# IC3Net/IC3Net

Hardware: AMD Instinct MI355X
Metric: env-steps/sec (agents x envs x steps), rollout hot path (higher is better)
Workload: dtype f32

## Files before the change

### ic3net_amd/csrc/bptt_kernels.hip

```cpp
#include <hip/hip_runtime.h>

#include <algorithm>
#include <vector>

#include "enc_bwd.hpp"
#include "ic3_common.hpp"
#include "ps_common.hpp"

extern "C" int ic3_lstm_gates_backward_given(const float* gates, float* xh, int ldx, const float* h_prev, const void* lstm_wp3_bwd,
                                             const float* c_prev, const float* dh, const float* dc, float* dgates, float* dc_prev,
                                             float* dbias_partials, int accumulate, float* dxh, const float* row_live,
                                             const float* row_keep, const float* dhead, const float* w_heads, int OT, int R, int H,
                                             ic3_stream stream);

namespace ic3 {

typedef float bp_f32x2 __attribute__((ext_vector_type(2)));
typedef float bp_f32x4 __attribute__((ext_vector_type(4)));
typedef float bp_f32x16 __attribute__((ext_vector_type(16)));

__device__ __forceinline__ __amdgpu_buffer_rsrc_t bp_rsrc(const void* base, long long bytes)
{
    const uint32_t n = bytes <= 0 ? 0u : (bytes > 0xffffffffll ? 0xffffffffu : (uint32_t)bytes);
    return __builtin_amdgcn_make_buffer_rsrc(const_cast<void*>(base), 0, n, 0x00020000);
// ... 493 lines not shown
        IC3_HIP(hipGetLastError());
        const int n3 = 2 * H * 4 * H;
        hipLaunchKernelGGL(wgrad_reduce_kernel, dim3((n3 + 255) / 256), dim3(256), 0, s, scratch, ks, n3, dW, accumulate);
        IC3_HIP(hipGetLastError());
        return ks;
    }
    const size_t lds = (size_t)2 * 16 * (2 * H + 128) * sizeof(float);
    if (H == 128) {
        IC3_HIP(ensure_dynamic_lds(reinterpret_cast<const void*>(lstm_wgrad_kernel<128>), lds));
        hipLaunchKernelGGL((lstm_wgrad_kernel<128>), dim3(ks, 4), dim3(256), lds, s, a);
    } else {
        IC3_HIP(ensure_dynamic_lds(reinterpret_cast<const void*>(lstm_wgrad_kernel<64>), lds));
        hipLaunchKernelGGL((lstm_wgrad_kernel<64>), dim3(ks, 2), dim3(256), lds, s, a);
    }
    IC3_HIP(hipGetLastError());
    const int n = 2 * H * 4 * H;
    hipLaunchKernelGGL(wgrad_reduce_kernel, dim3((n + 255) / 256), dim3(256), 0, s, scratch, ks, n, dW, accumulate);
    IC3_HIP(hipGetLastError());
    return ks;
}

extern "C" int ic3_bptt_backward_supported(const ic3_env* env, int H)
{
    using namespace ic3;
    if (!env || (H != 64 && H != 128 && H != 256) || env->dims.N > 64) return 0;
    EncBwdPlan pl;
    if (env->kind == IC3_ENV_PP) {
        const ic3_pp_cfg& c = env->pp;
        const int W = 2 * c.vision + 1;
        pl = enc_bwd_plan(c.E, env->dims.N, c.N + c.nprey, H, c.dim * c.dim, 2 * W * W);
    } else {
        const ic3_tj_cfg& c = env->tj;
        const int WW = env->dims.window * env->dims.window, hdr = c.vocab_type ? 4 : 2;
        pl = enc_bwd_plan(c.E, c.N, c.N, H, env->dims.grid_h * env->dims.grid_w, hdr + WW);
    }
    return pl.csplit ? 1 : 0;
}

namespace ic3 {
struct BpttSide {
    hipStream_t stream = nullptr;
    hipEvent_t fork = nullptr, join = nullptr;
};
static BpttSide* bptt_side()
{
    static BpttSide side[64];
    int dev = 0;
    if (hipGetDevice(&dev) != hipSuccess || dev < 0 || dev >= 64) return nullptr;
    BpttSide& sd = side[dev];
    if (!sd.stream) {
        if (hipStreamCreateWithFlags(&sd.stream, hipStreamNonBlocking) != hipSuccess) return nullptr;
        if (hipEventCreateWithFlags(&sd.fork, hipEventDisableTiming) != hipSuccess ||
            hipEventCreateWithFlags(&sd.join, hipEventDisableTiming) != hipSuccess)
            return nullptr;
    }
    return &sd;
}
}

extern "C" int ic3_bptt_first_chain_envs(int E, int N)
{
    if (E < 128 || N <= 0) return E;
    return (E / 2) & ~63;
}

extern "C" int ic3_bptt_backward(ic3_env* env, const ic3_bptt* b, ic3_stream stream)
{
    using namespace ic3;
    if (!env || !b) return fail(-22, "ic3_bptt_backward: null argument");
    if (b->struct_size != sizeof(ic3_bptt))
        return fail(-22, "ic3_bptt_backward: ic3_bptt has " + std::to_string(b->struct_size) + " bytes, this library's has " +
                             std::to_string(sizeof(ic3_bptt)) + " (header / library version mismatch)");
    const int T = b->T, E = b->E, N = b->N, H = b->H;
    if (T <= 0 || E <= 0 || N <= 0 || E != env->dims.E || N != env->dims.N)
        return fail(-22, "ic3_bptt_backward: T, E, N must be positive and E, N the handle's");
    if (!ic3_bptt_backward_supported(env, H)) return fail(-38, "ic3_bptt_backward: hid_size 64 / 128 / 256, <= 64 agents, a grid whose encoder backward runs in its partial-sums form");
    if (b->OT < 1 || b->OT > 16) return fail(-22, "ic3_bptt_backward: 1 <= OT <= 16");
    if (!b->gates || !b->hs || !b->cs || !b->dhead || !b->snaps || !b->lstm_wp3_bwd || !b->w_heads || !b->dh || !b->dc || !b->dxh ||
        !b->dbias_partials || !b->enc_work)
        return fail(-22, "ic3_bptt_backward: null argument");
    if (!b->comm_zero && (!b->c_weight || !b->dcw_partials)) return fail(-22, "ic3_bptt_backward: C.weight and its partials");
    if (b->dxh_step && (b->dxh_step < (long long)E * N * 2 * H || ic3_env_encode_backward_window_work(env, H) <= 0))
        return fail(-22, "ic3_bptt_backward: dxh_step >= E * N * 2 * hid_size, on a configuration with ic3_env_encode_backward_window");
    const long long R = (long long)E * N;
    hipStream_t s = (hipStream_t)stream;
    const int E1 = (b->two_chains && b->dxh_step) ? ic3_bptt_first_chain_envs(E, N) : E;
    const int nch = E1 < E ? 2 : 1;
    BpttSide* side = nch == 2 ? bptt_side() : nullptr;
    if (nch == 2 && !side) return fail(-12, "ic3_bptt_backward: no second stream");
    if (nch == 2) {
        IC3_HIP(hipEventRecord(side->fork, s));
        IC3_HIP(hipStreamWaitEvent(side->stream, side->fork, 0));
    }
    int enc_first = b->enc_first;
    for (int t = T - 1; t >= 0; --t) {
        for (int ch = 0; ch < nch; ++ch) {
            const int e0 = ch ? E1 : 0, Ec = ch ? E - E1 : E1;
            const size_t r0 = (size_t)e0 * N, Rc = (size_t)Ec * N;
            hipStream_t sc = ch ? side->stream : s;
            ic3_stream scv = (ic3_stream)sc;
            float* dh = b->dh + r0 * H;
            float* dc = b->dc + r0 * H;
            const bool detached = b->detach_gap > 0 && (t + 1) % b->detach_gap == 0;
            float* g = b->gates + ((size_t)t * R + r0) * 4 * H;
            float* dxh = b->dxh + (size_t)t * (size_t)b->dxh_step + r0 * 2 * H;
            if (b->gate_events && ch == 0) IC3_HIP(hipEventRecord((hipEvent_t)b->gate_events[2 * t], sc));
            int rc = ic3_lstm_gates_backward_given(g, nullptr, 0, nullptr, b->lstm_wp3_bwd, b->cs + ((size_t)t * R + r0) * H,
                                                   detached ? nullptr : dh, detached ? nullptr : dc, g,
                                                   dc, b->dbias_partials + (r0 / 64) * 4 * H, 1, dxh,
                                                   b->row_live ? b->row_live + (size_t)t * R + r0 : nullptr,
                                                   b->row_keep ? b->row_keep + (size_t)t * R + r0 : nullptr,
                                                   b->dhead + ((size_t)t * R + r0) * b->OT, b->w_heads, b->OT, (int)Rc, H, scv);
            if (rc < 0) return rc;
            if (b->gate_events && ch == 0) IC3_HIP(hipEventRecord((hipEvent_t)b->gate_events[2 * t + 1], sc));
            const float* out_scale = (b->row_keep && t > 0) ? b->row_keep + (size_t)(t - 1) * R + r0 : nullptr;
            float* dcw = b->dcw_partials;
            if (dcw && ch) dcw += (size_t)ic3_comm_backward_partials(E1, N) * H * H;
            rc = ic3_comm_backward(dxh, 2 * H, b->hs + ((size_t)t * R + r0) * H, (b->alive && b->alive[t]) ? b->alive[t] + r0 : nullptr,
                                   (b->gate && b->gate[t]) ? b->gate[t] + r0 : nullptr, b->c_weight, out_scale, dh, dcw, 1, Ec, N, H,
                                   b->mode_avg, b->comm_zero, scv);
            if (rc < 0) return rc;
        }
        if (b->dxh_step) continue;
        int rc = ic3_env_encode_backward_accumulate(env, b->snaps + (size_t)t * b->snap_words, b->dxh, 2 * H, H, b->enc_work,
                                                    enc_first, stream);
        if (rc < 0) return rc;
        enc_first = 0;
    }
    if (nch == 2) {
        IC3_HIP(hipEventRecord(side->join, side->stream));
        IC3_HIP(hipStreamWaitEvent(s, side->join, 0));
    }
    if (b->dxh_step)
        return ic3_env_encode_backward_window(env, b->snaps, b->snap_words, T, b->dxh, 2 * H, b->dxh_step, H, b->enc_work, enc_first,
                                              stream);
    return 0;
}

namespace ic3 {

struct RnnBwdArgs {
    const float* dh_in;
    const float* h;
    const float* dhead;
    const float* w_heads;
    const float* a2;
    const float* out_scale;
    float* dz;
    float* dh_out;
    float* db_part;
    int R, OT, tiles, accumulate;
};

template <int H>
__global__ __launch_bounds__(4 * H, (H <= 64) ? 2 : 1) void rnn_tanh_bwd_kernel(const RnnBwdArgs a)
{
    constexpr int NT = 4 * H, H4 = H / 4, LDA = H + 4, LDA4 = LDA / 4, CB = H / 32, RPP = NT / H4, PER = 64 / RPP;
    static_assert(RPP * PER == 64 && NT / 64 == 2 * CB, "tile split");
    IC3_DYNAMIC_LDS(float, smem);
    const bp_f32x4* const Bf4 = reinterpret_cast<const bp_f32x4*>(smem);
    float* const Dz = smem + H * H;
    bp_f32x4* const Dz4 = reinterpret_cast<bp_f32x4*>(Dz);
    float* const Wh = Dz + 64 * LDA;
    const bp_f32x4* const Wh4 = reinterpret_cast<const bp_f32x4*>(Wh);
    float* const Sd = Wh + 16 * H;
    const int tid = threadIdx.x, lane = tid & 63, w = tid >> 6, li = lane & 31, lh = lane >> 5;
    const int cb = w % CB, rb = w / CB;
    const int c4 = tid % H4, rg = tid / H4;
    const int OT = a.OT;
    for (int i = tid; i < H * H; i += NT) {
        const int k = i / H, col = i - k * H;
        smem[(((k >> 3) * 2 + ((k >> 2) & 1)) * H + col) * 4 + (k & 3)] = a.a2[i];
    }
    for (int i = tid; i < OT * H; i += NT) Wh[i] = a.w_heads[i];
    bp_f32x4 bsum = { 0.f, 0.f, 0.f, 0.f };
    __syncthreads();
    for (int tile = blockIdx.x; tile < a.tiles; tile += gridDim.x) {
        const long long r0 = (long long)tile * 64;
        const int rows = (a.R - r0) < 64 ? (int)(a.R - r0) : 64;
        const __amdgpu_buffer_rsrc_t rdi = bp_rsrc(a.dh_in ? a.dh_in + r0 * H : a.h, a.dh_in ? (long long)rows * H * 4 : 0);
        const __amdgpu_buffer_rsrc_t rh = bp_rsrc(a.h + r0 * H, (long long)rows * H * 4);
        const __amdgpu_buffer_rsrc_t rd = bp_rsrc(a.dhead + r0 * OT, (long long)rows * OT * 4);
        const __amdgpu_buffer_rsrc_t rz = bp_rsrc(a.dz + r0 * H, (long long)rows * H * 4);
        bp_f32x4 dv[PER], hv[PER];
#pragma unroll
        for (int i = 0; i < PER; ++i) {
            const int off = ((rg + RPP * i) * H + 4 * c4) * 4;
            dv[i] = bp_load4(rdi, off);
            hv[i] = bp_load4(rh, off);
        }
        for (int i = tid; i < 64 * OT; i += NT) Sd[i] = bp_load1(rd, i * 4);
        __syncthreads();
#pragma unroll
        for (int i = 0; i < PER; ++i) {
            const int row = rg + RPP * i;
            bp_f32x4 v = dv[i];
            for (int o = 0; o < OT; ++o) v += Sd[row * OT + o] * Wh4[o * H4 + c4];
            const bp_f32x4 z = v * (1.0f - hv[i] * hv[i]);
            bsum += z;
            Dz4[row * LDA4 + c4] = z;
            __builtin_amdgcn_raw_buffer_store_b128(__builtin_bit_cast(ps_u32x4, z), rz, (row * H + 4 * c4) * 4, 0, 0);
        }
        __syncthreads();
        bp_f32x16 acc;
#pragma unroll
        for (int i = 0; i < 16; ++i) acc[i] = 0.0f;
#pragma unroll 4
        for (int kb = 0; kb < H / 8; ++kb) {
            const bp_f32x4 a4 = Dz4[(32 * rb + li) * LDA4 + 2 * kb + lh];
// ... 246 lines not shown
```

### ic3net_amd/csrc/gates_bwd.hip

```cpp
#include <hip/hip_runtime.h>

#include "ic3_common.hpp"

namespace ic3 {

typedef float gb_f32x4 __attribute__((ext_vector_type(4)));
typedef float gb_f32x16 __attribute__((ext_vector_type(16)));
typedef unsigned int gb_u32x4 __attribute__((ext_vector_type(4)));

struct GatesBwdArgs {
    float* xh;
    const float* h_prev;
    const float* wq;
    const void* wq3;
    const float* bias;
    const float* c_prev;
    const float* dh;
    const float* dc;
    float* dgates;
    float* dc_prev;
    float* dbias;
    int ldx, R, accumulate;
    const void* wb3;
    float* dxh;
    const float* gates;
    const float* row_live;
    const float* row_keep;
    const float* dhead;
    const float* w_heads;
    int OT;
};

__device__ __forceinline__ __amdgpu_buffer_rsrc_t gb_rsrc(const void* base, long long bytes)
{
    const uint32_t n = bytes <= 0 ? 0u : (bytes > 0xffffffffll ? 0xffffffffu : (uint32_t)bytes);
    return __builtin_amdgcn_make_buffer_rsrc(const_cast<void*>(base), 0, n, 0x00020000);
}
__device__ __forceinline__ gb_f32x4 gb_load4(__amdgpu_buffer_rsrc_t r, int voff, int soff)
{
    return __builtin_bit_cast(gb_f32x4, __builtin_amdgcn_raw_buffer_load_b128(r, voff, soff, 0));
}
__device__ __forceinline__ float gb_load1(__amdgpu_buffer_rsrc_t r, int voff, int soff)
{
    return __builtin_bit_cast(float, __builtin_amdgcn_raw_buffer_load_b32(r, voff, soff, 0));
}
__device__ __forceinline__ void gb_store1(float v, __amdgpu_buffer_rsrc_t r, int voff, int soff)
{
    __builtin_amdgcn_raw_buffer_store_b32(__builtin_bit_cast(int, v), r, voff, soff, 0);
}

__device__ __forceinline__ void gb_mfma(gb_f32x16& acc, float x, float y)
{
    acc = __builtin_amdgcn_mfma_f32_32x32x2f32(x, y, acc, 0, 0, 0);
}

typedef __bf16 gb_bf16x2 __attribute__((ext_vector_type(2)));
typedef float gb_f32x2 __attribute__((ext_vector_type(2)));
__device__ __forceinline__ void gb_split_pair(gb_f32x2 x, unsigned& p1, unsigned& p2, unsigned& p3)
{
    const gb_bf16x2 h1 = __builtin_convertvector(x, gb_bf16x2);
    const gb_f32x2 r1 = x - __builtin_convertvector(h1, gb_f32x2);
    const gb_bf16x2 h2 = __builtin_convertvector(r1, gb_bf16x2);
    const gb_f32x2 r2 = r1 - __builtin_convertvector(h2, gb_f32x2);
    const gb_bf16x2 h3 = __builtin_convertvector(r2, gb_bf16x2);
    p1 = __builtin_bit_cast(unsigned, h1);
    p2 = __builtin_bit_cast(unsigned, h2);
    p3 = __builtin_bit_cast(unsigned, h3);
}
__device__ __forceinline__ void gb_split_frag(gb_f32x4 x0, gb_f32x4 x1, gb_u32x4 (&out)[3])
{
    unsigned p[3][4];
    gb_split_pair(gb_f32x2{ x0[0], x0[1] }, p[0][0], p[1][0], p[2][0]);
    gb_split_pair(gb_f32x2{ x0[2], x0[3] }, p[0][1], p[1][1], p[2][1]);
    gb_split_pair(gb_f32x2{ x1[0], x1[1] }, p[0][2], p[1][2], p[2][2]);
    gb_split_pair(gb_f32x2{ x1[2], x1[3] }, p[0][3], p[1][3], p[2][3]);
#pragma unroll
    for (int pl = 0; pl < 3; ++pl) out[pl] = gb_u32x4{ p[pl][0], p[pl][1], p[pl][2], p[pl][3] };
}
__device__ __forceinline__ void gb_mfma_bf16(gb_f32x16& acc, gb_u32x4 x, gb_u32x4 y)
{
    typedef __bf16 gb_bf16x8 __attribute__((ext_vector_type(8)));
    acc = __builtin_amdgcn_mfma_f32_32x32x16_bf16(__builtin_bit_cast(gb_bf16x8, x), __builtin_bit_cast(gb_bf16x8, y), acc, 0, 0, 0);
}

template <int H, int SPLIT = 0, int GIVEN = 0>
__global__ __launch_bounds__(2 * H, (H <= 128) ? 2 : 1) void lstm_gates_bwd_kernel(const GatesBwdArgs a)
{
    static_assert(!GIVEN || SPLIT == 1, "recorded gates: the split instantiation (its dx product)");
    constexpr int K = 2 * H, LDA = K + 4, LDA4 = LDA / 4, NT = 2 * H, KB = K / 8, K4 = K / 4, RING = 8;
    static_assert(KB % 2 == 0 && KB >= 4, "K / 8 must be even");
    IC3_DYNAMIC_LDS(float, smem);
    float* const As = smem;
    gb_f32x4* const As4 = reinterpret_cast<gb_f32x4*>(smem);
    float* const slb = As + 64 * LDA;
    float* const sdh = slb + 4 * H;
    const int tid = threadIdx.x, lane = tid & 63, w = tid >> 6, li = lane & 31, lh = lane >> 5;
    const int col = 32 * w + li;
    const long long r0 = (long long)blockIdx.x * 64;
    const int rows = (int)((a.R - r0) < 64 ? (a.R - r0) : 64);

    if constexpr (GIVEN != 0) {
        if (a.dhead) {
            const __amdgpu_buffer_rsrc_t rdd = gb_rsrc(a.dhead + r0 * a.OT, (long long)rows * a.OT * 4);
            for (int idx = tid; idx < 64 * 16; idx += NT) {
                const int row = idx >> 4, o = idx & 15;
                sdh[idx] = o < a.OT ? gb_load1(rdd, (row * a.OT + o) * 4, 0) : 0.0f;
            }
        }
        if (a.xh && a.h_prev) {
            const __amdgpu_buffer_rsrc_t rx = gb_rsrc(a.xh + r0 * a.ldx, ((long long)(rows - 1) * a.ldx + K) * 4);
            const __amdgpu_buffer_rsrc_t rhp = gb_rsrc(a.h_prev + r0 * H, (long long)rows * H * 4);
            constexpr int H4 = H / 4, PERH = 64 * H4 / NT;
#pragma unroll
            for (int i = 0; i < PERH; ++i) {
                const int idx = tid + i * NT, row = idx / H4, c4 = idx - row * H4;
                gb_f32x4 v = gb_load4(rhp, (row * H + 4 * c4) * 4, 0);
                if (a.row_live) v *= (row < rows ? a.row_live[r0 + row] : 0.0f);
                __builtin_amdgcn_raw_buffer_store_b128(__builtin_bit_cast(gb_u32x4, v), rx, (row * a.ldx + H + 4 * c4) * 4, 0, 0);
            }
        }
    } else {
        const __amdgpu_buffer_rsrc_t rx = gb_rsrc(a.xh + r0 * a.ldx, ((long long)(rows - 1) * a.ldx + K) * 4);
        constexpr int PER = 64 * K4 / NT;
        const __amdgpu_buffer_rsrc_t rhp = gb_rsrc(a.h_prev ? a.h_prev + r0 * H : a.xh, a.h_prev ? (long long)rows * H * 4 : 0);
        const bool from_h = a.h_prev != nullptr;
        gb_f32x4 v[PER];
#pragma unroll
        for (int i = 0; i < PER; ++i) {
            const int idx = tid + i * NT, row = idx / K4, c4 = idx - row * K4;
            if (from_h && c4 >= H / 4) {
                v[i] = gb_load4(rhp, (row * H + 4 * c4 - H) * 4, 0);
                __builtin_amdgcn_raw_buffer_store_b128(__builtin_bit_cast(gb_u32x4, v[i]), rx, (row * a.ldx + 4 * c4) * 4, 0, 0);
            } else {
                v[i] = gb_load4(rx, (row * a.ldx + 4 * c4) * 4, 0);
            }
        }
        if (tid < H) reinterpret_cast<gb_f32x4*>(slb)[tid] = reinterpret_cast<const gb_f32x4*>(a.bias)[tid];
#pragma unroll
        for (int i = 0; i < PER; ++i) {
            const int idx = tid + i * NT, row = idx / K4, c4 = idx - row * K4;
            As4[row * LDA4 + c4] = v[i];
        }
    }
    const int voff = (4 * lh * H + col) * 4;
    float cold[2][16];
    const __amdgpu_buffer_rsrc_t rc = gb_rsrc(a.c_prev + r0 * H, (long long)rows * H * 4);
    if constexpr (SPLIT == 0) {
#pragma unroll
        for (int rt = 0; rt < 2; ++rt)
#pragma unroll
            for (int reg = 0; reg < 16; ++reg)
                cold[rt][reg] = gb_load1(rc, voff, (32 * rt + (reg & 3) + 8 * (reg >> 2)) * H * 4);
    }
    gb_f32x16 acc[2][4];
#pragma unroll
    for (int rt = 0; rt < 2; ++rt)
#pragma unroll
        for (int gt = 0; gt < 4; ++gt)
#pragma unroll
            for (int i = 0; i < 16; ++i) acc[rt][gt][i] = 0.0f;
    if constexpr (GIVEN != 0) {
    } else if constexpr (SPLIT != 0) {
        constexpr int KB16 = K / 16, NWv = H / 32;
        const __amdgpu_buffer_rsrc_t rg3 = gb_rsrc(a.wq3, (long long)3 * K * 4 * H * 2);
        const int g3lane = (w * 64 + lane) * 16;
        constexpr int GSTRIDE = NWv * 64 * 16;
        auto wq3 = [&](int pl, int kb, int gt) {
            return __builtin_amdgcn_raw_buffer_load_b128(rg3, g3lane, ((pl * KB16 + kb) * 4 + gt) * GSTRIDE, 0);
        };
        gb_u32x4 bq[3][4];
#pragma unroll
        for (int pl = 0; pl < 3; ++pl)
#pragma unroll
            for (int gt = 0; gt < 4; ++gt) bq[pl][gt] = wq3(pl, 0, gt);
        __syncthreads();
        auto block3 = [&](auto refill_c, int kb) {
            constexpr bool REFILL = decltype(refill_c)::value;
            gb_u32x4 ap[2][3];
            {
                const gb_f32x4* s0 = As4 + li * LDA4 + 4 * kb + 2 * lh;
                const gb_f32x4* s1 = As4 + (32 + li) * LDA4 + 4 * kb + 2 * lh;
                gb_split_frag(s0[0], s0[1], ap[0]);
                gb_split_frag(s1[0], s1[1], ap[1]);
            }
#pragma unroll
            for (int pb = 0; pb < 3; ++pb)
#pragma unroll
                for (int gt = 0; gt < 4; ++gt) {
#pragma unroll
                    for (int pa = 2; pa >= 0; --pa) {
                        gb_mfma_bf16(acc[0][gt], ap[0][pa], bq[pb][gt]);
                        gb_mfma_bf16(acc[1][gt], ap[1][pa], bq[pb][gt]);
                    }
                    if constexpr (REFILL) bq[pb][gt] = wq3(pb, kb + 1, gt);
                    __builtin_amdgcn_sched_barrier(0);
                }
        };
#pragma unroll 1
        for (int kb = 0; kb < KB16 - 1; ++kb) block3(std::true_type{}, kb);
        block3(std::false_type{}, KB16 - 1);
        __builtin_amdgcn_sched_barrier(0);
    } else {
        const __amdgpu_buffer_rsrc_t rgw = gb_rsrc(a.wq, (long long)K * 4 * H * 4);
        const int glane = (4 * lh * H + col) * 16;
        auto wq = [&](int kb, int j) { return gb_load4(rgw, glane, (8 * kb + j) * (H * 16)); };
        gb_f32x4 wk[RING];
    #pragma unroll
        for (int i = 0; i < RING; ++i) wk[i] = wq(i >> 2, i & 3);
        __syncthreads();
        auto block = [&](auto sb_c, auto refill_c, int kb) {
            constexpr int SB = decltype(sb_c)::value;
            constexpr bool REFILL = decltype(refill_c)::value;
            const gb_f32x4 a0 = As4[li * LDA4 + 2 * kb + lh];
            const gb_f32x4 a1 = As4[(32 + li) * LDA4 + 2 * kb + lh];
    #pragma unroll
            for (int j = 0; j < 4; ++j) {
    #pragma unroll
                for (int gt = 0; gt < 4; ++gt) {
                    gb_mfma(acc[0][gt], a0[j], wk[SB + j][gt]);
                    gb_mfma(acc[1][gt], a1[j], wk[SB + j][gt]);
                }
                if constexpr (REFILL) wk[SB + j] = wq(kb + RING / 4, j);
                __builtin_amdgcn_sched_barrier(0);
            }
        };
        constexpr std::integral_constant<int, 0> s0{};
        constexpr std::integral_constant<int, 4> s1{};
    #pragma unroll 1
        for (int kb = 0; kb < KB - 2; kb += 2) {
            block(s0, std::true_type{}, kb);
            block(s1, std::true_type{}, kb + 1);
        }
        block(s0, std::false_type{}, KB - 2);
        block(s1, std::false_type{}, KB - 1);
        __builtin_amdgcn_sched_barrier(0);
    }

    const float bi = GIVEN ? 0.f : slb[col], bf = GIVEN ? 0.f : slb[H + col], bg = GIVEN ? 0.f : slb[2 * H + col], bo = GIVEN ? 0.f : slb[3 * H + col];
    const bool dx = SPLIT != 0 && a.dxh != nullptr;
    float keep_g[2][16], keep_o[2][16];
    const bool heads_in = GIVEN != 0 && a.dhead != nullptr;
    if (dx || heads_in) __syncthreads();
    float wh[16] = {};
    if constexpr (GIVEN != 0) {
        if (heads_in) {
            const __amdgpu_buffer_rsrc_t rwh = gb_rsrc(a.w_heads, (long long)a.OT * H * 4);
#pragma unroll
            for (int o = 0; o < 16; ++o) wh[o] = gb_load1(rwh, (o * H + col) * 4, 0);
        }
    }
    const long long nrec = (long long)rows * H * 4;
    const __amdgpu_buffer_rsrc_t rdh = gb_rsrc(a.dh ? a.dh + r0 * H : a.c_prev, a.dh ? nrec : 0);
    const __amdgpu_buffer_rsrc_t rdc = gb_rsrc(a.dc ? a.dc + r0 * H : a.c_prev, a.dc ? nrec : 0);
    const __amdgpu_buffer_rsrc_t rdp = gb_rsrc(a.dc_prev + r0 * H, nrec);
    const __amdgpu_buffer_rsrc_t rdg = gb_rsrc(a.dgates + r0 * 4 * H, 4 * nrec);
    const int goff = (4 * lh * 4 * H + col) * 4;
    const __amdgpu_buffer_rsrc_t rgin = gb_rsrc(GIVEN ? a.gates + r0 * 4 * H : a.c_prev, GIVEN ? 4 * nrec : 0);
    const bool cuts = GIVEN != 0 && (a.row_live != nullptr || a.row_keep != nullptr);
    const __amdgpu_buffer_rsrc_t rlive = gb_rsrc(a.row_live ? a.row_live + r0 : a.c_prev, a.row_live ? (long long)rows * 4 : 0);
    const __amdgpu_buffer_rsrc_t rkeep = gb_rsrc(a.row_keep ? a.row_keep + r0 : a.c_prev, a.row_keep ? (long long)rows * 4 : 0);
    float si = 0.f, sf = 0.f, sg = 0.f, so = 0.f;
#pragma unroll
    for (int rt = 0; rt < 2; ++rt) {
        float dhv[16], dcv[16], gin[GIVEN ? 4 : 1][16];
#pragma unroll
        for (int reg = 0; reg < 16; ++reg) {
            const int lc = 32 * rt + (reg & 3) + 8 * (reg >> 2);
            dhv[reg] = gb_load1(rdh, voff, lc * H * 4);
            dcv[reg] = gb_load1(rdc, voff, lc * H * 4);
            if constexpr (SPLIT != 0) cold[rt][reg] = gb_load1(rc, voff, lc * H * 4);
            if constexpr (GIVEN != 0) {
#pragma unroll
                for (int k = 0; k < 4; ++k) gin[k][reg] = gb_load1(rgin, goff, lc * 4 * H * 4 + k * H * 4);
            }
        }
#pragma unroll
        for (int reg = 0; reg < 16; ++reg) {
            const int lc = 32 * rt + (reg & 3) + 8 * (reg >> 2);
            float i, f, gt, o;
            if constexpr (GIVEN != 0) {
                i = gin[0][reg], f = gin[1][reg], gt = gin[2][reg], o = gin[3][reg];
                if (heads_in) {
                    const gb_f32x4* dr = reinterpret_cast<const gb_f32x4*>(sdh + (lc + 4 * lh) * 16);
                    float s = dhv[reg];
#pragma unroll
                    for (int q = 0; q < 4; ++q) {
                        if (4 * q >= a.OT) break;
                        const gb_f32x4 dv = dr[q];
                        s = __builtin_fmaf(dv[0], wh[4 * q], s);
                        s = __builtin_fmaf(dv[1], wh[4 * q + 1], s);
                        s = __builtin_fmaf(dv[2], wh[4 * q + 2], s);
                        s = __builtin_fmaf(dv[3], wh[4 * q + 3], s);
                    }
                    dhv[reg] = s;
                }
                if (cuts) {
                    const int lrow = lc + 4 * lh;
                    if (a.row_live) cold[rt][reg] *= gb_load1(rlive, lrow * 4, 0);
                    if (a.row_keep) dcv[reg] *= gb_load1(rkeep, lrow * 4, 0);
                }
            } else {
                i = fast_sigmoid(acc[rt][0][reg] + bi), f = fast_sigmoid(acc[rt][1][reg] + bf);
                gt = fast_tanh(acc[rt][2][reg] + bg), o = fast_sigmoid(acc[rt][3][reg] + bo);
            }
            const float c0 = cold[rt][reg];
            const float tc = fast_tanh(__builtin_fmaf(f, c0, i * gt));
            const float dct = dcv[reg] + dhv[reg] * o * (1.0f - tc * tc);
            const float di = dct * gt * i * (1.0f - i), df = dct * c0 * f * (1.0f - f);
            const float dg = dct * i * (1.0f - gt * gt), dO = dhv[reg] * tc * o * (1.0f - o);
            gb_store1(di, rdg, goff, lc * 4 * H * 4);
            gb_store1(df, rdg, goff, lc * 4 * H * 4 + H * 4);
            gb_store1(dg, rdg, goff, lc * 4 * H * 4 + 2 * H * 4);
            gb_store1(dO, rdg, goff, lc * 4 * H * 4 + 3 * H * 4);
            gb_store1(dct * f, rdp, voff, lc * H * 4);
            if constexpr (SPLIT != 0) {
                if (dx) {
                    const int lr = lc + 4 * lh;
                    As[lr * LDA + col] = di;
                    As[lr * LDA + H + col] = df;
                    keep_g[rt][reg] = dg;
                    keep_o[rt][reg] = dO;
                }
            }
            si += di;
            sf += df;
            sg += dg;
            so += dO;
        }
    }
    if constexpr (SPLIT != 0) {
        if (dx) {
            constexpr int KB16B = 4 * H / 16, NCT = 2 * H / 32, KBH = K / 16;
            const __amdgpu_buffer_rsrc_t rwb = gb_rsrc(a.wb3, (long long)3 * 4 * H * 2 * H * 2);
            const int wu = __builtin_amdgcn_readfirstlane(w);
            auto wb = [&](int pl, int kg, int ct) __attribute__((always_inline)) {
                return __builtin_amdgcn_raw_buffer_load_b128(rwb, lane * 16, ((pl * KB16B + kg) * NCT + 2 * wu + ct) * 1024, 0);
            };
            gb_u32x4 bq2[3][2];
#pragma unroll
            for (int pl = 0; pl < 3; ++pl)
#pragma unroll
                for (int ct = 0; ct < 2; ++ct) bq2[pl][ct] = wb(pl, 0, ct);
#pragma unroll
            for (int rt = 0; rt < 2; ++rt)
#pragma unroll
                for (int ct = 0; ct < 2; ++ct)
#pragma unroll
                    for (int i = 0; i < 16; ++i) acc[rt][ct][i] = 0.0f;
            auto blockdx = [&](int kb, int kg) __attribute__((always_inline)) {
                gb_u32x4 ap[2][3];
                const gb_f32x4* s0 = As4 + li * LDA4 + 4 * kb + 2 * lh;
                const gb_f32x4* s1 = As4 + (32 + li) * LDA4 + 4 * kb + 2 * lh;
                gb_split_frag(s0[0], s0[1], ap[0]);
                gb_split_frag(s1[0], s1[1], ap[1]);
#pragma unroll
                for (int pb = 0; pb < 3; ++pb)
#pragma unroll
                    for (int ct = 0; ct < 2; ++ct) {
#pragma unroll
                        for (int pa = 2; pa >= 0; --pa) {
                            gb_mfma_bf16(acc[0][ct], ap[0][pa], bq2[pb][ct]);
                            gb_mfma_bf16(acc[1][ct], ap[1][pa], bq2[pb][ct]);
                        }
                        if (kg + 1 < KB16B) bq2[pb][ct] = wb(pb, kg + 1, ct);
                        __builtin_amdgcn_sched_barrier(0);
                    }
            };
            __syncthreads();
#pragma unroll 1
            for (int kb = 0; kb < KBH; ++kb) blockdx(kb, kb);
            __syncthreads();
#pragma unroll
            for (int rt = 0; rt < 2; ++rt)
#pragma unroll
                for (int reg = 0; reg < 16; ++reg) {
                    const int lr = 32 * rt + (reg & 3) + 8 * (reg >> 2) + 4 * lh;
                    As[lr * LDA + col] = keep_g[rt][reg];
                    As[lr * LDA + H + col] = keep_o[rt][reg];
                }
            __syncthreads();
#pragma unroll 1
            for (int kb = 0; kb < KBH; ++kb) blockdx(kb, KBH + kb);
            const __amdgpu_buffer_rsrc_t rdx = gb_rsrc(a.dxh + r0 * K, (long long)rows * K * 4);
#pragma unroll
            for (int rt = 0; rt < 2; ++rt)
#pragma unroll
                for (int ct = 0; ct < 2; ++ct)
#pragma unroll
                    for (int reg = 0; reg < 16; ++reg) {
                        const int lr = 32 * rt + (reg & 3) + 8 * (reg >> 2) + 4 * lh;
                        gb_store1(acc[rt][ct][reg], rdx, (lr * K + 64 * w + 32 * ct + li) * 4, 0);
                    }
        }
    }
    if (a.dbias) {
        si += __shfl_xor(si, 32);
        sf += __shfl_xor(sf, 32);
        sg += __shfl_xor(sg, 32);
        so += __shfl_xor(so, 32);
        if (lh == 0) {
            float* d = a.dbias + (size_t)blockIdx.x * 4 * H + col;
            if (a.accumulate) {
                d[0] += si;
                d[H] += sf;
                d[2 * H] += sg;
                d[3 * H] += so;
            } else {
                d[0] = si;
                d[H] = sf;
                d[2 * H] = sg;
                d[3 * H] = so;
            }
        }
    }
}

}

extern "C" int ic3_lstm_gates_backward_supported(int H) { return H == 64 || H == 128 || H == 256; }

static int gates_backward_impl(float* xh, int ldx, const float* h_prev, const float* lstm_wp, const void* lstm_wp3, const float* bias,
                               const float* c_prev, const float* dh, const float* dc, float* dgates, float* dc_prev,
                               float* dbias_partials, int accumulate, const void* wb3, float* dxh, int R, int H, ic3_stream stream,
                               const float* gates = nullptr, const float* row_live = nullptr, const float* row_keep = nullptr,
                               const float* dhead = nullptr, const float* w_heads = nullptr, int OT = 0);

extern "C" int ic3_lstm_gates_backward(float* xh, int ldx, const float* h_prev, const float* lstm_wp, const void* lstm_wp3, const float* bias, const float* c_prev,
                                       const float* dh, const float* dc, float* dgates, float* dc_prev, float* dbias_partials,
                                       int accumulate, int R, int H, ic3_stream stream)
{
    return gates_backward_impl(xh, ldx, h_prev, lstm_wp, lstm_wp3, bias, c_prev, dh, dc, dgates, dc_prev, dbias_partials, accumulate,
                               nullptr, nullptr, R, H, stream);
}

extern "C" int ic3_lstm_gates_backward_dx(float* xh, int ldx, const float* h_prev, const float* lstm_wp, const void* lstm_wp3,
                                          const void* lstm_wp3_bwd, const float* bias, const float* c_prev, const float* dh,
                                          const float* dc, float* dgates, float* dc_prev, float* dbias_partials, int accumulate,
                                          float* dxh, int R, int H, ic3_stream stream)
{
    if (!lstm_wp3 || !lstm_wp3_bwd || !dxh)
        return ic3::fail(-22, "ic3_lstm_gates_backward_dx: needs the split planes of both products (lstm_wp3, lstm_wp3_bwd) and dxh");
    if (H != 64 && H != 128) return ic3::fail(-38, "ic3_lstm_gates_backward_dx: hid_size 64 / 128");
    return gates_backward_impl(xh, ldx, h_prev, lstm_wp, lstm_wp3, bias, c_prev, dh, dc, dgates, dc_prev, dbias_partials, accumulate,
                               lstm_wp3_bwd, dxh, R, H, stream);
}

extern "C" int ic3_lstm_gates_backward_given(const float* gates, float* xh, int ldx, const float* h_prev, const void* lstm_wp3_bwd,
                                             const float* c_prev, const float* dh, const float* dc, float* dgates, float* dc_prev,
                                             float* dbias_partials, int accumulate, float* dxh, const float* row_live,
                                             const float* row_keep, const float* dhead, const float* w_heads, int OT, int R, int H,
                                             ic3_stream stream)
{
    if (!gates) return ic3::fail(-22, "ic3_lstm_gates_backward_given: null gates");
    if ((dhead == nullptr) != (w_heads == nullptr) || (dhead && (OT < 1 || OT > 16)))
        return ic3::fail(-22, "ic3_lstm_gates_backward_given: dhead [R][OT] and w_heads [OT][H] come together, 1 <= OT <= 16");
    if (row_keep && !dc) return ic3::fail(-22, "ic3_lstm_gates_backward_given: row_keep scales dc");
    if ((lstm_wp3_bwd == nullptr) != (dxh == nullptr))
        return ic3::fail(-22, "ic3_lstm_gates_backward_given: lstm_wp3_bwd and dxh come together");
    if (H != 64 && H != 128 && H != 256) return ic3::fail(-38, "ic3_lstm_gates_backward_given: hid_size 64 / 128 / 256");
    if ((xh == nullptr) != (h_prev == nullptr))
        return ic3::fail(-22, "ic3_lstm_gates_backward_given: xh and h_prev come together (the copy into xh's h half) or not at all");
    return gates_backward_impl(xh, xh ? ldx : 2 * H, h_prev, nullptr, nullptr, nullptr, c_prev, dh, dc, dgates, dc_prev, dbias_partials,
                               accumulate, lstm_wp3_bwd, dxh, R, H, stream, gates, row_live, row_keep, dhead, w_heads, OT);
}

static int gates_backward_impl(float* xh, int ldx, const float* h_prev, const float* lstm_wp, const void* lstm_wp3, const float* bias,
                               const float* c_prev, const float* dh, const float* dc, float* dgates, float* dc_prev,
                               float* dbias_partials, int accumulate, const void* wb3, float* dxh, int R, int H, ic3_stream stream,
                               const float* gates, const float* row_live, const float* row_keep, const float* dhead,
                               const float* w_heads, int OT)
{
    using namespace ic3;
    if ((!gates && (!xh || !lstm_wp || !bias)) || !c_prev || (!dh && !gates) || !dgates || !dc_prev || R <= 0)
        return fail(-22, "ic3_lstm_gates_backward: null argument");
    if (!ic3_lstm_gates_backward_supported(H)) return fail(-38, "ic3_lstm_gates_backward: needs hid_size 64 / 128 / 256");
    if (ldx < 2 * H || (ldx & 3)) return fail(-22, "ic3_lstm_gates_backward: ldx must be a multiple of 4, >= 2 * hid_size");
    if ((long long)R * (ldx > 4 * H ? ldx : 4 * H) * 4 >= (1ll << 32))
        return fail(-22, "ic3_lstm_gates_backward: R * 4H floats must stay below 4 GB (32-bit buffer offsets)");
    const GatesBwdArgs a{ xh, h_prev, lstm_wp, lstm_wp3, bias, c_prev, dh, dc, dgates, dc_prev, dbias_partials, ldx, R, accumulate, wb3, dxh, gates, row_live, row_keep, dhead, w_heads, OT };
    const int tiles = (R + 63) / 64;
    const size_t lds = ((size_t)64 * (2 * H + 4) + 4 * H + (gates ? 64 * 16 : 0)) * sizeof(float);
    hipStream_t s = (hipStream_t)stream;
    if (gates) {
        if (H == 256) {
            IC3_HIP(ensure_dynamic_lds(reinterpret_cast<const void*>(lstm_gates_bwd_kernel<256, 1, 1>), lds));
            hipLaunchKernelGGL((lstm_gates_bwd_kernel<256, 1, 1>), dim3(tiles), dim3(512), lds, s, a);
        } else if (H == 128) {
            IC3_HIP(ensure_dynamic_lds(reinterpret_cast<const void*>(lstm_gates_bwd_kernel<128, 1, 1>), lds));
            hipLaunchKernelGGL((lstm_gates_bwd_kernel<128, 1, 1>), dim3(tiles), dim3(256), lds, s, a);
        } else {
            IC3_HIP(ensure_dynamic_lds(reinterpret_cast<const void*>(lstm_gates_bwd_kernel<64, 1, 1>), lds));
            hipLaunchKernelGGL((lstm_gates_bwd_kernel<64, 1, 1>), dim3(tiles), dim3(128), lds, s, a);
        }
        IC3_HIP(hipGetLastError());
        return tiles;
    }
#define IC3_GB(h)                                                                                                       \
    case h:                                                                                                             \
        if (lstm_wp3) {                                                                                                 \
            IC3_HIP(ensure_dynamic_lds(reinterpret_cast<const void*>(lstm_gates_bwd_kernel<h, 1>), lds));               \
            hipLaunchKernelGGL((lstm_gates_bwd_kernel<h, 1>), dim3(tiles), dim3(2 * h), lds, s, a);                     \
        } else {                                                                                                        \
            IC3_HIP(ensure_dynamic_lds(reinterpret_cast<const void*>(lstm_gates_bwd_kernel<h, 0>), lds));               \
            hipLaunchKernelGGL((lstm_gates_bwd_kernel<h, 0>), dim3(tiles), dim3(2 * h), lds, s, a);                     \
        }                                                                                                               \
        break;
    switch (H) {
        IC3_GB(64)
        IC3_GB(128)
        IC3_GB(256)
    }
#undef IC3_GB
    IC3_HIP(hipGetLastError());
    return tiles;
}
```

Before: 280.8 million.

## Restructure recorded-gates LSTM backward into vectorized elementwise pass plus bf16x3 dx GEMM

Splits the recorded-gates path of the LSTM gates backward into its own device function. The elementwise part now uses row-major float4 loads and stores instead of scalar MFMA-fragment-layout accesses, and stages head weights in LDS. It then computes dx with a bf16 three-plane split MFMA product, staging dgates planes in LDS one gate quarter at a time. It also adds error-path stream joining and rejects detach_gap combined with row_keep. The aim is to cut scattered scalar memory traffic in the backward pass, at the cost of more LDS use and extra barriers.

```diff
diff --git a/ic3net_amd/csrc/bptt_kernels.hip b/ic3net_amd/csrc/bptt_kernels.hip
--- a/ic3net_amd/csrc/bptt_kernels.hip
+++ b/ic3net_amd/csrc/bptt_kernels.hip
@@ -599,6 +599,7 @@
     if (!b->comm_zero && (!b->c_weight || !b->dcw_partials)) return fail(-22, "ic3_bptt_backward: C.weight and its partials");
     if (b->dxh_step && (b->dxh_step < (long long)E * N * 2 * H || ic3_env_encode_backward_window_work(env, H) <= 0))
         return fail(-22, "ic3_bptt_backward: dxh_step >= E * N * 2 * hid_size, on a configuration with ic3_env_encode_backward_window");
+    if (b->detach_gap > 0 && b->row_keep) return fail(-22, "ic3_bptt_backward: detach_gap > 0 together with row_keep");
     const long long R = (long long)E * N;
     hipStream_t s = (hipStream_t)stream;
     const int E1 = (b->two_chains && b->dxh_step) ? ic3_bptt_first_chain_envs(E, N) : E;
@@ -609,6 +610,10 @@
         IC3_HIP(hipEventRecord(side->fork, s));
         IC3_HIP(hipStreamWaitEvent(side->stream, side->fork, 0));
     }
+    auto leave = [&](int rc) {
+        if (nch == 2 && hipEventRecord(side->join, side->stream) == hipSuccess) (void)hipStreamWaitEvent(s, side->join, 0);
+        return rc;
+    };
     int enc_first = b->enc_first;
     for (int t = T - 1; t >= 0; --t) {
         for (int ch = 0; ch < nch; ++ch) {
@@ -621,27 +626,29 @@
             const bool detached = b->detach_gap > 0 && (t + 1) % b->detach_gap == 0;
             float* g = b->gates + ((size_t)t * R + r0) * 4 * H;
             float* dxh = b->dxh + (size_t)t * (size_t)b->dxh_step + r0 * 2 * H;
-            if (b->gate_events && ch == 0) IC3_HIP(hipEventRecord((hipEvent_t)b->gate_events[2 * t], sc));
+            if (b->gate_events && ch == 0 && hipEventRecord((hipEvent_t)b->gate_events[2 * t], sc) != hipSuccess)
+                return leave(fail(-5, "ic3_bptt_backward: hipEventRecord(gate_events)"));
             int rc = ic3_lstm_gates_backward_given(g, nullptr, 0, nullptr, b->lstm_wp3_bwd, b->cs + ((size_t)t * R + r0) * H,
                                                    detached ? nullptr : dh, detached ? nullptr : dc, g,
                                                    dc, b->dbias_partials + (r0 / 64) * 4 * H, 1, dxh,
                                                    b->row_live ? b->row_live + (size_t)t * R + r0 : nullptr,
                                                    b->row_keep ? b->row_keep + (size_t)t * R + r0 : nullptr,
                                                    b->dhead + ((size_t)t * R + r0) * b->OT, b->w_heads, b->OT, (int)Rc, H, scv);
-            if (rc < 0) return rc;
-            if (b->gate_events && ch == 0) IC3_HIP(hipEventRecord((hipEvent_t)b->gate_events[2 * t + 1], sc));
+            if (rc < 0) return leave(rc);
+            if (b->gate_events && ch == 0 && hipEventRecord((hipEvent_t)b->gate_events[2 * t + 1], sc) != hipSuccess)
+                return leave(fail(-5, "ic3_bptt_backward: hipEventRecord(gate_events)"));
             const float* out_scale = (b->row_keep && t > 0) ? b->row_keep + (size_t)(t - 1) * R + r0 : nullptr;
             float* dcw = b->dcw_partials;
             if (dcw && ch) dcw += (size_t)ic3_comm_backward_partials(E1, N) * H * H;
             rc = ic3_comm_backward(dxh, 2 * H, b->hs + ((size_t)t * R + r0) * H, (b->alive && b->alive[t]) ? b->alive[t] + r0 : nullptr,
                                    (b->gate && b->gate[t]) ? b->gate[t] + r0 : nullptr, b->c_weight, out_scale, dh, dcw, 1, Ec, N, H,
                                    b->mode_avg, b->comm_zero, scv);
-            if (rc < 0) return rc;
+            if (rc < 0) return leave(rc);
         }
         if (b->dxh_step) continue;
         int rc = ic3_env_encode_backward_accumulate(env, b->snaps + (size_t)t * b->snap_words, b->dxh, 2 * H, H, b->enc_work,
                                                     enc_first, stream);
-        if (rc < 0) return rc;
+        if (rc < 0) return leave(rc);
         enc_first = 0;
     }
     if (nch == 2) {
diff --git a/ic3net_amd/csrc/gates_bwd.hip b/ic3net_amd/csrc/gates_bwd.hip
--- a/ic3net_amd/csrc/gates_bwd.hip
+++ b/ic3net_amd/csrc/gates_bwd.hip
@@ -83,43 +83,247 @@
     acc = __builtin_amdgcn_mfma_f32_32x32x16_bf16(__builtin_bit_cast(gb_bf16x8, x), __builtin_bit_cast(gb_bf16x8, y), acc, 0, 0, 0);
 }
 
-template <int H, int SPLIT = 0, int GIVEN = 0>
-__global__ __launch_bounds__(2 * H, (H <= 128) ? 2 : 1) void lstm_gates_bwd_kernel(const GatesBwdArgs a)
-{
-    static_assert(!GIVEN || SPLIT == 1, "recorded gates: the split instantiation (its dx product)");
+struct GivenLds {
+    int main_bytes, sdh_off, swh_off, total;
+};
+__host__ __device__ constexpr GivenLds gb_given_lds(int H)
+{
+    const int planes = 3 * 64 * (2 * H + 16), ctile = 64 * (2 * H + 4) * 4, red = 8 * 4 * H * 4;
+    const int m = planes > ctile ? (planes > red ? planes : red) : (ctile > red ? ctile : red);
+    return GivenLds{ m, m / 4, m / 4 + 64 * 16, m + 64 * 16 * 4 + 16 * H * 4 };
+}
+
+template <int H>
+__device__ __forceinline__ void gates_bwd_given(const GatesBwdArgs& a, float* smem)
+{
+    typedef unsigned int gb_u32x2 __attribute__((ext_vector_type(2)));
+    constexpr int K = 2 * H, NT = 2 * H, H4 = H / 4, K4 = K / 4, ITEMS = 8, LDC = K + 4;
+    constexpr int RS = 2 * H + 16, PSZ = 64 * RS;
+    constexpr GivenLds L = gb_given_lds(H);
+    static_assert(64 * H4 == ITEMS * NT && NT / H4 == 8, "eight rows per pass, eight passes");
+    char* const planes = reinterpret_cast<char*>(smem);
+    float* const Cs = smem;
+    float* const red = smem;
+    float* const sdh = smem + L.sdh_off;
+    gb_f32x4* const swh4 = reinterpret_cast<gb_f32x4*>(smem + L.swh_off);
+    const int tid = threadIdx.x, lane = tid & 63, w = tid >> 6, li = lane & 31, lh = lane >> 5;
+    const int c4 = tid % H4, rs = tid / H4;
+    const long long r0 = (long long)blockIdx.x * 64;
+    const int rows = (int)((a.R - r0) < 64 ? (a.R - r0) : 64);
+    const bool heads_in = a.dhead != nullptr;
+    const bool dx = a.dxh != nullptr;
+
+    if (heads_in) {
+        const __amdgpu_buffer_rsrc_t rdd = gb_rsrc(a.dhead + r0 * a.OT, (long long)rows * a.OT * 4);
+        for (int idx = tid; idx < 64 * 16; idx += NT) {
+            const int row = idx >> 4, o = idx & 15;
+            sdh[idx] = o < a.OT ? gb_load1(rdd, (row * a.OT + o) * 4, 0) : 0.0f;
+        }
+        const __amdgpu_buffer_rsrc_t rwh = gb_rsrc(a.w_heads, (long long)a.OT * H * 4);
+        for (int idx = tid; idx < 16 * H4; idx += NT) swh4[idx] = gb_load4(rwh, idx * 16, 0);
+    }
+    if (a.xh && a.h_prev) {
+        const __amdgpu_buffer_rsrc_t rx = gb_rsrc(a.xh + r0 * a.ldx, ((long long)(rows - 1) * a.ldx + K) * 4);
+        const __amdgpu_buffer_rsrc_t rhp = gb_rsrc(a.h_prev + r0 * H, (long long)rows * H * 4);
+#pragma unroll
+        for (int it = 0; it < ITEMS; ++it) {
+            const int row = rs + 8 * it;
+            gb_f32x4 v = gb_load4(rhp, (row * H + 4 * c4) * 4, 0);
+            if (a.row_live) v *= (row < rows ? a.row_live[r0 + row] : 0.0f);
+            __builtin_amdgcn_raw_buffer_store_b128(__builtin_bit_cast(gb_u32x4, v), rx, (row * a.ldx + H + 4 * c4) * 4, 0, 0);
+        }
+    }
+    if (heads_in) __syncthreads();
+
+    const long long nrec = (long long)rows * H * 4;
+    const __amdgpu_buffer_rsrc_t rc = gb_rsrc(a.c_prev + r0 * H, nrec);
+    const __amdgpu_buffer_rsrc_t rdh = gb_rsrc(a.dh ? a.dh + r0 * H : a.c_prev, a.dh ? nrec : 0);
+    const __amdgpu_buffer_rsrc_t rdc = gb_rsrc(a.dc ? a.dc + r0 * H : a.c_prev, a.dc ? nrec : 0);
+    const __amdgpu_buffer_rsrc_t rdp = gb_rsrc(a.dc_prev + r0 * H, nrec);
+    const __amdgpu_buffer_rsrc_t rdg = gb_rsrc(a.dgates + r0 * 4 * H, 4 * nrec);
+    const __amdgpu_buffer_rsrc_t rgin = gb_rsrc(a.gates + r0 * 4 * H, 4 * nrec);
+    const __amdgpu_buffer_rsrc_t rlive = gb_rsrc(a.row_live ? a.row_live + r0 : a.c_prev, a.row_live ? (long long)rows * 4 : 0);
+    const __amdgpu_buffer_rsrc_t rkeep = gb_rsrc(a.row_keep ? a.row_keep + r0 : a.c_prev, a.row_keep ? (long long)rows * 4 : 0);
+    const int voff = (rs * H + 4 * c4) * 4, goff = (rs * 4 * H + 4 * c4) * 4;
+    auto put = [&](int row, gb_f32x4 v) __attribute__((always_inline)) {
+        unsigned p[3][2];
+        gb_split_pair(gb_f32x2{ v[0], v[1] }, p[0][0], p[1][0], p[2][0]);
+        gb_split_pair(gb_f32x2{ v[2], v[3] }, p[0][1], p[1][1], p[2][1]);
+#pragma unroll
+        for (int pl = 0; pl < 3; ++pl) *reinterpret_cast<gb_u32x2*>(planes + pl * PSZ + row * RS + 8 * c4) = gb_u32x2{ p[pl][0], p[pl][1] };
+    };
+    float sum[4][4] = {};
+    gb_f32x4 nxt[ITEMS];
+#pragma unroll
+    for (int b = 0; b < ITEMS; b += 2) {
+        gb_f32x4 gin[2][4], c0v[2], dhv[2], dcv[2];
+        float live[2] = { 1.0f, 1.0f }, keep[2] = { 1.0f, 1.0f };
+#pragma unroll
+        for (int j = 0; j < 2; ++j) {
+            const int it = b + j;
+#pragma unroll
+            for (int g = 0; g < 4; ++g) gin[j][g] = gb_load4(rgin, goff, it * 8 * 4 * H * 4 + g * H * 4);
+            c0v[j] = gb_load4(rc, voff, it * 8 * H * 4);
+            dhv[j] = gb_load4(rdh, voff, it * 8 * H * 4);
+            dcv[j] = gb_load4(rdc, voff, it * 8 * H * 4);
+            if (a.row_live) live[j] = gb_load1(rlive, rs * 4, it * 32);
+            if (a.row_keep) keep[j] = gb_load1(rkeep, rs * 4, it * 32);
+        }
+        __builtin_amdgcn_sched_barrier(0);
+#pragma unroll
+        for (int j = 0; j < 2; ++j) {
+            const int it = b + j, row = rs + 8 * it;
+            if (heads_in) {
+                const gb_f32x4* dr = reinterpret_cast<const gb_f32x4*>(sdh + row * 16);
+#pragma unroll
+                for (int q = 0; q < 4; ++q) {
+                    if (4 * q >= a.OT) break;
+                    const gb_f32x4 dv = dr[q];
+#pragma unroll
+                    for (int u = 0; u < 4; ++u) {
+                        const gb_f32x4 wv = swh4[(4 * q + u) * H4 + c4];
+#pragma unroll
+                        for (int e = 0; e < 4; ++e) dhv[j][e] = __builtin_fmaf(dv[u], wv[e], dhv[j][e]);
+                    }
+                }
+            }
+            gb_f32x4 dg4[4], dcp;
+#pragma unroll
+            for (int e = 0; e < 4; ++e) {
+                const float i = gin[j][0][e], f = gin[j][1][e], gt = gin[j][2][e], o = gin[j][3][e];
+                float c0 = c0v[j][e], dcin = dcv[j][e];
+                if (a.row_live) c0 *= live[j];
+                if (a.row_keep) dcin *= keep[j];
+                const float dhe = dhv[j][e];
+                const float tc = fast_tanh(__builtin_fmaf(f, c0, i * gt));
+                const float dct = dcin + dhe * o * (1.0f - tc * tc);
+                const float di = dct * gt * i * (1.0f - i), df = dct * c0 * f * (1.0f - f);
+                const float dg = dct * i * (1.0f - gt * gt), dO = dhe * tc * o * (1.0f - o);
+                dg4[0][e] = di, dg4[1][e] = df, dg4[2][e] = dg, dg4[3][e] = dO;
+                dcp[e] = dct * f;
+            }
+#pragma unroll
+            for (int g = 0; g < 4; ++g) {
+                __builtin_amdgcn_raw_buffer_store_b128(__builtin_bit_cast(gb_u32x4, dg4[g]), rdg, goff, it * 8 * 4 * H * 4 + g * H * 4, 0);
+#pragma unroll
+                for (int e = 0; e < 4; ++e) sum[g][e] += dg4[g][e];
+            }
+            __builtin_amdgcn_raw_buffer_store_b128(__builtin_bit_cast(gb_u32x4, dcp), rdp, voff, it * 8 * H * 4, 0);
+            if (dx) put(row, dg4[0]);
+            nxt[it] = dg4[1];
+        }
+        __builtin_amdgcn_sched_barrier(0);
+    }
+#pragma unroll
+    for (int g = 0; g < 4; ++g)
+#pragma unroll
+        for (int e = 0; e < 4; ++e) IC3_OPAQUE_VGPR(sum[g][e]);
+
+    if (dx) {
+        constexpr int KB16B = 4 * H / 16, NCT = 2 * H / 32, KBQ = H / 16;
+        const __amdgpu_buffer_rsrc_t rwb = gb_rsrc(a.wb3, (long long)3 * 4 * H * 2 * H * 2);
+        const int wu = __builtin_amdgcn_readfirstlane(w);
+        auto wb = [&](int pl, int kg, int ct) __attribute__((always_inline)) {
+            return __builtin_amdgcn_raw_buffer_load_b128(rwb, lane * 16, ((pl * KB16B + kg) * NCT + 2 * wu + ct) * 1024, 0);
+        };
+        gb_u32x4 bq2[3][2];
+#pragma unroll
+        for (int pl = 0; pl < 3; ++pl)
+#pragma unroll
+            for (int ct = 0; ct < 2; ++ct) bq2[pl][ct] = wb(pl, 0, ct);
+        gb_f32x16 acc[2][2];
+#pragma unroll
+        for (int rt = 0; rt < 2; ++rt)
+#pragma unroll
+            for (int ct = 0; ct < 2; ++ct)
+#pragma unroll
+                for (int i = 0; i < 16; ++i) acc[rt][ct][i] = 0.0f;
+        const char* const afrag = planes + li * RS + 16 * lh;
+        auto blockdx = [&](int kb, int kg) __attribute__((always_inline)) {
+            gb_u32x4 ap[2][3];
+#pragma unroll
+            for (int rt = 0; rt < 2; ++rt)
+#pragma unroll
+                for (int pa = 0; pa < 3; ++pa)
+                    ap[rt][pa] = *reinterpret_cast<const gb_u32x4*>(afrag + pa * PSZ + 32 * rt * RS + 32 * kb);
+#pragma unroll
+            for (int pb = 0; pb < 3; ++pb)
+#pragma unroll
+                for (int ct = 0; ct < 2; ++ct) {
+#pragma unroll
+                    for (int pa = 2; pa >= 0; --pa) {
+                        gb_mfma_bf16(acc[0][ct], ap[0][pa], bq2[pb][ct]);
+                        gb_mfma_bf16(acc[1][ct], ap[1][pa], bq2[pb][ct]);
+                    }
+                    if (kg + 1 < KB16B) bq2[pb][ct] = wb(pb, kg + 1, ct);
+                    __builtin_amdgcn_sched_barrier(0);
+                }
+        };
+#pragma unroll 1
+        for (int q = 0; q < 4; ++q) {
+            __syncthreads();
+#pragma unroll 1
+            for (int kb = 0; kb < KBQ; ++kb) blockdx(kb, q * KBQ + kb);
+            if (q == 3) break;
+            __syncthreads();
+#pragma unroll
+            for (int it = 0; it < ITEMS; ++it) put(rs + 8 * it, nxt[it]);
+            if (q < 2) {
+#pragma unroll
+                for (int it = 0; it < ITEMS; ++it) nxt[it] = gb_load4(rdg, goff, it * 8 * 4 * H * 4 + (q + 2) * H * 4);
+            }
+        }
+        __syncthreads();
+#pragma unroll
+        for (int rt = 0; rt < 2; ++rt)
+#pragma unroll
+            for (int ct = 0; ct < 2; ++ct)
+#pragma unroll
+                for (int reg = 0; reg < 16; ++reg) {
+                    const int lr = 32 * rt + (reg & 3) + 8 * (reg >> 2) + 4 * lh;
+                    Cs[lr * LDC + 64 * w + 32 * ct + li] = acc[rt][ct][reg];
+                }
+        __syncthreads();
+        const __amdgpu_buffer_rsrc_t rdx = gb_rsrc(a.dxh + r0 * K, (long long)rows * K * 4);
+#pragma unroll
+        for (int i = 0; i < 64 * K4 / NT; ++i) {
+            const int idx = tid + i * NT, row = idx / K4, c = idx - row * K4;
+            const gb_f32x4 v = *reinterpret_cast<const gb_f32x4*>(Cs + row * LDC + 4 * c);
+            __builtin_amdgcn_raw_buffer_store_b128(__builtin_bit_cast(gb_u32x4, v), rdx, (row * K + 4 * c) * 4, 0, 0);
+        }
+    }
+    if (a.dbias) {
+        __syncthreads();
+#pragma unroll
+        for (int g = 0; g < 4; ++g)
+            *reinterpret_cast<gb_f32x4*>(red + rs * 4 * H + g * H + 4 * c4) = gb_f32x4{ sum[g][0], sum[g][1], sum[g][2], sum[g][3] };
+        __syncthreads();
+#pragma unroll
+        for (int i = 0; i < 2; ++i) {
+            const int c = tid + i * NT;
+            float v = red[c];
+#pragma unroll
+            for (int s = 1; s < 8; ++s) v += red[s * 4 * H + c];
+            float* d = a.dbias + (size_t)blockIdx.x * 4 * H + c;
+            *d = a.accumulate ? *d + v : v;
+        }
+    }
+}
+
+template <int H, int SPLIT>
+__device__ __forceinline__ void gates_bwd_recompute(const GatesBwdArgs& a, float* smem)
+{
     constexpr int K = 2 * H, LDA = K + 4, LDA4 = LDA / 4, NT = 2 * H, KB = K / 8, K4 = K / 4, RING = 8;
     static_assert(KB % 2 == 0 && KB >= 4, "K / 8 must be even");
-    IC3_DYNAMIC_LDS(float, smem);
     float* const As = smem;
     gb_f32x4* const As4 = reinterpret_cast<gb_f32x4*>(smem);
     float* const slb = As + 64 * LDA;
-    float* const sdh = slb + 4 * H;
     const int tid = threadIdx.x, lane = tid & 63, w = tid >> 6, li = lane & 31, lh = lane >> 5;
     const int col = 32 * w + li;
     const long long r0 = (long long)blockIdx.x * 64;
     const int rows = (int)((a.R - r0) < 64 ? (a.R - r0) : 64);
 
-    if constexpr (GIVEN != 0) {
-        if (a.dhead) {
-            const __amdgpu_buffer_rsrc_t rdd = gb_rsrc(a.dhead + r0 * a.OT, (long long)rows * a.OT * 4);
-            for (int idx = tid; idx < 64 * 16; idx += NT) {
-                const int row = idx >> 4, o = idx & 15;
-                sdh[idx] = o < a.OT ? gb_load1(rdd, (row * a.OT + o) * 4, 0) : 0.0f;
-            }
-        }
-        if (a.xh && a.h_prev) {
-            const __amdgpu_buffer_rsrc_t rx = gb_rsrc(a.xh + r0 * a.ldx, ((long long)(rows - 1) * a.ldx + K) * 4);
-            const __amdgpu_buffer_rsrc_t rhp = gb_rsrc(a.h_prev + r0 * H, (long long)rows * H * 4);
-            constexpr int H4 = H / 4, PERH = 64 * H4 / NT;
-#pragma unroll
-            for (int i = 0; i < PERH; ++i) {
-                const int idx = tid + i * NT, row = idx / H4, c4 = idx - row * H4;
-                gb_f32x4 v = gb_load4(rhp, (row * H + 4 * c4) * 4, 0);
-                if (a.row_live) v *= (row < rows ? a.row_live[r0 + row] : 0.0f);
-                __builtin_amdgcn_raw_buffer_store_b128(__builtin_bit_cast(gb_u32x4, v), rx, (row * a.ldx + H + 4 * c4) * 4, 0, 0);
-            }
-        }
-    } else {
+    {
         const __amdgpu_buffer_rsrc_t rx = gb_rsrc(a.xh + r0 * a.ldx, ((long long)(rows - 1) * a.ldx + K) * 4);
         constexpr int PER = 64 * K4 / NT;
         const __amdgpu_buffer_rsrc_t rhp = gb_rsrc(a.h_prev ? a.h_prev + r0 * H : a.xh, a.h_prev ? (long long)rows * H * 4 : 0);
@@ -159,8 +363,7 @@
         for (int gt = 0; gt < 4; ++gt)
 #pragma unroll
             for (int i = 0; i < 16; ++i) acc[rt][gt][i] = 0.0f;
-    if constexpr (GIVEN != 0) {
-    } else if constexpr (SPLIT != 0) {
+    if constexpr (SPLIT != 0) {
         constexpr int KB16 = K / 16, NWv = H / 32;
         const __amdgpu_buffer_rsrc_t rg3 = gb_rsrc(a.wq3, (long long)3 * K * 4 * H * 2);
         const int g3lane = (w * 64 + lane) * 16;
@@ -236,73 +439,32 @@
         __builtin_amdgcn_sched_barrier(0);
     }
 
-    const float bi = GIVEN ? 0.f : slb[col], bf = GIVEN ? 0.f : slb[H + col], bg = GIVEN ? 0.f : slb[2 * H + col], bo = GIVEN ? 0.f : slb[3 * H + col];
+    const float bi = slb[col], bf = slb[H + col], bg = slb[2 * H + col], bo = slb[3 * H + col];
     const bool dx = SPLIT != 0 && a.dxh != nullptr;
     float keep_g[2][16], keep_o[2][16];
-    const bool heads_in = GIVEN != 0 && a.dhead != nullptr;
-    if (dx || heads_in) __syncthreads();
-    float wh[16] = {};
-    if constexpr (GIVEN != 0) {
-        if (heads_in) {
-            const __amdgpu_buffer_rsrc_t rwh = gb_rsrc(a.w_heads, (long long)a.OT * H * 4);
-#pragma unroll
-            for (int o = 0; o < 16; ++o) wh[o] = gb_load1(rwh, (o * H + col) * 4, 0);
-        }
-    }
+    if (dx) __syncthreads();
     const long long nrec = (long long)rows * H * 4;
     const __amdgpu_buffer_rsrc_t rdh = gb_rsrc(a.dh ? a.dh + r0 * H : a.c_prev, a.dh ? nrec : 0);
     const __amdgpu_buffer_rsrc_t rdc = gb_rsrc(a.dc ? a.dc + r0 * H : a.c_prev, a.dc ? nrec : 0);
     const __amdgpu_buffer_rsrc_t rdp = gb_rsrc(a.dc_prev + r0 * H, nrec);
     const __amdgpu_buffer_rsrc_t rdg = gb_rsrc(a.dgates + r0 * 4 * H, 4 * nrec);
     const int goff = (4 * lh * 4 * H + col) * 4;
-    const __amdgpu_buffer_rsrc_t rgin = gb_rsrc(GIVEN ? a.gates + r0 * 4 * H : a.c_prev, GIVEN ? 4 * nrec : 0);
-    const bool cuts = GIVEN != 0 && (a.row_live != nullptr || a.row_keep != nullptr);
-    const __amdgpu_buffer_rsrc_t rlive = gb_rsrc(a.row_live ? a.row_live + r0 : a.c_prev, a.row_live ? (long long)rows * 4 : 0);
-    const __amdgpu_buffer_rsrc_t rkeep = gb_rsrc(a.row_keep ? a.row_keep + r0 : a.c_prev, a.row_keep ? (long long)rows * 4 : 0);
     float si = 0.f, sf = 0.f, sg = 0.f, so = 0.f;
 #pragma unroll
     for (int rt = 0; rt < 2; ++rt) {
-        float dhv[16], dcv[16], gin[GIVEN ? 4 : 1][16];
+        float dhv[16], dcv[16];
 #pragma unroll
         for (int reg = 0; reg < 16; ++reg) {
             const int lc = 32 * rt + (reg & 3) + 8 * (reg >> 2);
             dhv[reg] = gb_load1(rdh, voff, lc * H * 4);
             dcv[reg] = gb_load1(rdc, voff, lc * H * 4);
             if constexpr (SPLIT != 0) cold[rt][reg] = gb_load1(rc, voff, lc * H * 4);
-            if constexpr (GIVEN != 0) {
-#pragma unroll
-                for (int k = 0; k < 4; ++k) gin[k][reg] = gb_load1(rgin, goff, lc * 4 * H * 4 + k * H * 4);
-            }
         }
 #pragma unroll
         for (int reg = 0; reg < 16; ++reg) {
             const int lc = 32 * rt + (reg & 3) + 8 * (reg >> 2);
-            float i, f, gt, o;
-            if constexpr (GIVEN != 0) {
-                i = gin[0][reg], f = gin[1][reg], gt = gin[2][reg], o = gin[3][reg];
-                if (heads_in) {
-                    const gb_f32x4* dr = reinterpret_cast<const gb_f32x4*>(sdh + (lc + 4 * lh) * 16);
-                    float s = dhv[reg];
-#pragma unroll
-                    for (int q = 0; q < 4; ++q) {
-                        if (4 * q >= a.OT) break;
-                        const gb_f32x4 dv = dr[q];
-                        s = __builtin_fmaf(dv[0], wh[4 * q], s);
-                        s = __builtin_fmaf(dv[1], wh[4 * q + 1], s);
-                        s = __builtin_fmaf(dv[2], wh[4 * q + 2], s);
-                        s = __builtin_fmaf(dv[3], wh[4 * q + 3], s);
-                    }
-                    dhv[reg] = s;
-                }
-                if (cuts) {
-                    const int lrow = lc + 4 * lh;
-                    if (a.row_live) cold[rt][reg] *= gb_load1(rlive, lrow * 4, 0);
-                    if (a.row_keep) dcv[reg] *= gb_load1(rkeep, lrow * 4, 0);
-                }
-            } else {
-                i = fast_sigmoid(acc[rt][0][reg] + bi), f = fast_sigmoid(acc[rt][1][reg] + bf);
-                gt = fast_tanh(acc[rt][2][reg] + bg), o = fast_sigmoid(acc[rt][3][reg] + bo);
-            }
+            const float i = fast_sigmoid(acc[rt][0][reg] + bi), f = fast_sigmoid(acc[rt][1][reg] + bf);
+            const float gt = fast_tanh(acc[rt][2][reg] + bg), o = fast_sigmoid(acc[rt][3][reg] + bo);
             const float c0 = cold[rt][reg];
             const float tc = fast_tanh(__builtin_fmaf(f, c0, i * gt));
             const float dct = dcv[reg] + dhv[reg] * o * (1.0f - tc * tc);
@@ -415,6 +577,15 @@
     }
 }
 
+template <int H, int SPLIT = 0, int GIVEN = 0>
+__global__ __launch_bounds__(2 * H, (H <= 128) ? 2 : 1) void lstm_gates_bwd_kernel(const GatesBwdArgs a)
+{
+    static_assert(!GIVEN || SPLIT == 1, "recorded gates: the split instantiation (its dx product)");
+    IC3_DYNAMIC_LDS(float, smem);
+    if constexpr (GIVEN != 0) gates_bwd_given<H>(a, smem);
+    else gates_bwd_recompute<H, SPLIT>(a, smem);
+}
+
 }
 
 extern "C" int ic3_lstm_gates_backward_supported(int H) { return H == 64 || H == 128 || H == 256; }
@@ -479,7 +650,7 @@
         return fail(-22, "ic3_lstm_gates_backward: R * 4H floats must stay below 4 GB (32-bit buffer offsets)");
     const GatesBwdArgs a{ xh, h_prev, lstm_wp, lstm_wp3, bias, c_prev, dh, dc, dgates, dc_prev, dbias_partials, ldx, R, accumulate, wb3, dxh, gates, row_live, row_keep, dhead, w_heads, OT };
     const int tiles = (R + 63) / 64;
-    const size_t lds = ((size_t)64 * (2 * H + 4) + 4 * H + (gates ? 64 * 16 : 0)) * sizeof(float);
+    const size_t lds = gates ? (size_t)gb_given_lds(H).total : ((size_t)64 * (2 * H + 4) + 4 * H) * sizeof(float);
     hipStream_t s = (hipStream_t)stream;
     if (gates) {
         if (H == 256) {
```

Result: no change. 282.0 million (median of 2 runs) (+0.4%).
